# nintendops/DynamicFusion_Body

Measured on AMD Instinct MI355X. Metric: Mvoxels/s TSDF fusion + GN-iters/s warp solve, 256³ grid, 1/2/4/8 GPU, higher is better.
Workload: dtype f64 geometry / f32 volume

## Files before the change

dynamicfusion_body_amd/_lib.py:

```python
import ctypes
import os
import re

_PKG = os.path.dirname(os.path.abspath(__file__))
LIB_PATH = os.environ.get("DFH_LIB_PATH") or os.path.join(_PKG, "libdfusion_hip.so")
HEADER_PATH = os.path.join(os.path.dirname(_PKG), "include", "dfusion_hip.h")

F32, F64 = 0, 1
ABI_VERSION = 8

_c_double_p = ctypes.POINTER(ctypes.c_double)
_c_int_p = ctypes.POINTER(ctypes.c_int)
_vp = ctypes.c_void_p
_int = ctypes.c_int
_dbl = ctypes.c_double


class Problem(ctypes.Structure):
    _fields_ = [("sample_pos", _vp), ("sample_nrm", _vp), ("nbr", _vp), ("weights", _vp), ("corr", _vp), ("valid", _vp),
                ("n_samples", _int), ("knn", _int),
                ("node_dq", _vp), ("node_pos", _vp), ("node_w", _vp), ("node_nbr", _vp), ("n_nodes", _int),
                ("lw_dq", _dbl * 8), ("rw", _dbl), ("huber_delta", _dbl),
                ("row_ptr", _vp), ("col", _vp), ("n_blocks", _int), ("vals", _vp), ("rhs", _vp), ("cost_count", _vp),
                ("blk_upper", _vp), ("n_upper", _int),
# ... 13 lines not shown
                ("global_lm", _dbl), ("global_xi_out", _vp), ("global_scratch", _vp), ("global_scratch_bytes", ctypes.c_size_t)]


class Slab(ctypes.Structure):
    _fields_ = [("res", _int * 3), ("x0", _int), ("x1", _int)]


class Volume(ctypes.Structure):
    _fields_ = [("tsdf", _vp), ("tsdf_w", _vp), ("dtype", _int), ("slab", Slab)]


class Live(ctypes.Structure):
    _fields_ = [("data", _vp), ("dtype", _int), ("res", _int * 3)]


class VolumeTerm(ctypes.Structure):
    _fields_ = [("live", Live), ("value_to_vox", _dbl), ("band", _dbl), ("max_dist", _dbl), ("min_grad", _dbl)]


class DepthViews(ctypes.Structure):
    _fields_ = [("n_views", _int), ("depth", ctypes.POINTER(_vp)), ("depth_dtype", _int), ("H", _int), ("W", _int),
                ("K", _dbl * 9), ("Kinv", _dbl * 9), ("lw", _c_double_p), ("scale", _dbl), ("center", _dbl * 3), ("tsdf_res", _int)]


class Nodes(ctypes.Structure):
    _fields_ = [("pos", _vp), ("dq", _vp), ("w", _vp), ("n_nodes", _int), ("knn", _int)]


_problem_p = ctypes.POINTER(Problem)
_frame_p = ctypes.POINTER(Frame)
_slab_p = ctypes.POINTER(Slab)
_volume_p = ctypes.POINTER(Volume)
_term_p = ctypes.POINTER(VolumeTerm)
STRUCTS = {"dfh_gn_problem": Problem, "dfh_gn_frame": Frame, "dfh_gn_solve_params": SolveParams, "dfh_slab": Slab,
           "dfh_volume": Volume, "dfh_live": Live, "dfh_depth_views": DepthViews, "dfh_nodes": Nodes,
           "dfh_gn_volume_term": VolumeTerm}

_SIGNATURES = {
    "dfh_version": (_int, []),
    "dfh_last_error": (ctypes.c_char_p, []),
    "dfh_stream_synchronize": (_int, [_vp]),
    "dfh_set_option": (_int, [ctypes.c_char_p, ctypes.c_long]),
    "dfh_get_option": (ctypes.c_long, [ctypes.c_char_p]),
    "dfh_integrate_workspace_bytes": (ctypes.c_size_t, [_int, _int, _int, _slab_p]),
    "dfh_integrate_multi_workspace_bytes": (ctypes.c_size_t, [_int]),
    "dfh_integrate_depth": (_int, [_volume_p, ctypes.POINTER(DepthViews), _dbl, _dbl, _c_double_p, _vp, ctypes.c_size_t, _vp]),
    "dfh_integrate_depth_path": (_int, [_int, _slab_p, _int, _int, _int]),
    "dfh_integrate_depth_ocl": (_int, [_volume_p, _vp, _int, _int, ctypes.POINTER(ctypes.c_float), ctypes.POINTER(ctypes.c_float), ctypes.c_float, ctypes.c_float, _vp]),
    "dfh_fuse_volume_rigid": (_int, [_volume_p, ctypes.POINTER(Live), _c_double_p, _dbl, _dbl, _vp]),
    "dfh_dqb_workspace_bytes": (ctypes.c_size_t, [_slab_p]),
    "dfh_dqb_workspace_bytes_cached": (ctypes.c_size_t, [_slab_p, _int, _int, _int]),
    "dfh_fuse_volume_dqb": (_int, [_volume_p, ctypes.POINTER(Live), ctypes.POINTER(Nodes), _c_double_p, _dbl, _dbl, _vp, ctypes.c_size_t, _int, _vp]),
    "dfh_integrate_depth_dqb": (_int, [_volume_p, ctypes.POINTER(DepthViews), ctypes.POINTER(Nodes), _c_double_p, _dbl, _dbl, _int, _vp,
                                      ctypes.c_size_t, _int, _vp]),
    "dfh_residual_rigid": (_int, [_vp, _vp, _vp, _int, _c_double_p, _vp, _vp]),
    "dfh_gn_build_rigid": (_int, [_vp, _vp, _vp, _vp, _int, _c_double_p, _vp, _vp]),
    "dfh_residual_data": (_int, [_vp, _vp, _vp, _vp, _int, _int, _vp, _vp, _vp, _int, _c_double_p, _vp, _vp]),
    "dfh_residual_reg": (_int, [_vp, _int, _int, _vp, _vp, _vp, _dbl, _vp, _vp]),
    "dfh_warp_points": (_int, [_vp, _vp, _vp, _int, _int, _vp, _vp, _vp, _int, _c_double_p, _vp, _vp, _vp]),
    "dfh_closest_correspondences": (_int, [_vp, _vp, _int, _vp, _int, _int, _dbl, _vp, _vp, _vp, _vp]),
    "dfh_nearest_points": (_int, [_vp, _int, _vp, _int, _vp, _vp, _vp]),
    "dfh_graph_unsupported": (_int, [_vp, _int, _vp, _int, _vp, _vp, _int, _vp, _vp]),
    "dfh_dq_blend_points": (_int, [_vp, _int, _vp, _int, _vp, _vp, _vp, _int, _vp, _vp]),
    "dfh_radius_sample_workspace_bytes": (ctypes.c_size_t, [ctypes.c_long]),
    "dfh_radius_sample": (_int, [_vp, ctypes.c_long, _dbl, _vp, ctypes.c_long, ctypes.POINTER(ctypes.c_long), _c_int_p, _vp,
                                 ctypes.c_size_t, _vp]),
    "dfh_sample_knn": (_int, [_vp, _int, _vp, _vp, _int, _int, _vp, _vp, _vp]),
    "dfh_dqb_skip_layout": (_int, [_slab_p, _c_int_p, _int, _int, ctypes.POINTER(ctypes.c_size_t)]),
    "dfh_dqb_build_candidates": (_int, [_slab_p, _vp, _int, _int, _vp, ctypes.c_size_t, _vp]),
    "dfh_sample_knn_bricks": (_int, [_vp, _int, _vp, _vp, _int, _int, _slab_p, _vp, ctypes.c_size_t, _vp, _vp, _vp]),
    "dfh_permute_samples": (_int, [_vp, _int, _int, _vp, _vp, _vp, _vp, _vp, _vp, _vp, _vp, _vp]),
    "dfh_gn_partial_doubles": (ctypes.c_size_t, [_int]),
    "dfh_gn_views_bytes": (ctypes.c_size_t, [_int, _int, _int, _int]),
    "dfh_gn_pack_views": (_int, [_vp, _int, ctypes.POINTER(ctypes.c_void_p), _int, _int, _int, _c_double_p, _vp]),
    "dfh_gn_associate": (_int, [_problem_p, _frame_p, _vp]),
    "dfh_gn_associate_volume": (_int, [_problem_p, _term_p, _vp]),
    "dfh_gn_build": (_int, [_problem_p, _frame_p, _vp]),
    "dfh_gn_build_volume": (_int, [_problem_p, _term_p, _vp]),
    "dfh_gn_solve": (_int, [_problem_p, _frame_p, ctypes.POINTER(SolveParams), _vp]),
    "dfh_gn_solve_volume": (_int, [_problem_p, _term_p, ctypes.POINTER(SolveParams), _vp]),
    "dfh_gn_pack_upper": (_int, [_vp, _vp, _vp, _vp, _int, _int, _int, _vp, _vp]),
    "dfh_gn_unpack_upper": (_int, [_vp, _vp, _vp, _vp, _int, _int, _int, _vp, _vp]),
    "dfh_gn_sort_workspace_bytes": (ctypes.c_size_t, [_int]),
    "dfh_gn_sort_samples": (_int, [_vp, _vp, _vp, _vp, _int, _int, _int, _vp, _vp, _vp, _vp, _vp, _vp, _vp, ctypes.c_size_t, _vp]),
    "dfh_gn_tile_samples": (_int, []),
    "dfh_gn_plan_count": (_int, [_vp, _int, _int, _vp, _vp, _vp]),
    "dfh_gn_plan_workspace_bytes": (ctypes.c_size_t, [_int, _int]),
    "dfh_gn_plan_build": (_int, [_vp, _int, _int, _int, _vp, _int, _vp, _vp, _int, _vp, _vp, _vp, _vp, _vp, _vp, _vp, _vp,
                                 ctypes.c_size_t, _vp]),
    "dfh_pcg_workspace_bytes": (ctypes.c_size_t, [_int, _int]),
    "dfh_pcg_solve": (_int, [_vp, _vp, _vp, _vp, _int, _int, _dbl, _dbl, _vp, _vp, ctypes.c_size_t, _vp]),
    "dfh_pcg_solve_update": (_int, [_vp, _vp, _vp, _vp, _int, _int, _dbl, _dbl, _vp, _vp, ctypes.c_size_t, _vp, _dbl, _vp]),
    "dfh_pcg_set_mode": (_int, [_int]),
    "dfh_pcg_path": (_int, [_int]),
    "dfh_pcg_status": (_int, [_vp, ctypes.POINTER(ctypes.c_long)]),
    "dfh_pcg_status_peek": (_int, [_vp, ctypes.POINTER(ctypes.c_long)]),
    "dfh_apply_twist": (_int, [_vp, _vp, _int, _dbl, _vp]),
    "dfh_relax_twists": (_int, [_vp, _int, _dbl, _vp]),
    "dfh_gn_global_sampled_bytes": (ctypes.c_size_t, [_int, _int]),
    "dfh_gn_global_sampled": (_int, [_problem_p, _frame_p, _int, _dbl, _int, _vp, _vp, _vp, ctypes.c_size_t, _vp]),
    "dfh_gn_global_sampled_volume": (_int, [_problem_p, _term_p, _int, _dbl, _int, _vp, _vp, _vp, ctypes.c_size_t, _vp]),
    "dfh_gn_global_apply": (_int, [_vp, _dbl, _int, _vp, _vp, _vp]),
    "dfh_gn_global_step_bytes": (ctypes.c_size_t, []),
    "dfh_gn_global_step": (_int, [_vp, _int, _vp, _int, _dbl, _vp, _vp, _vp, ctypes.c_size_t, _vp]),
    "dfh_surface_workspace_bytes": (ctypes.c_size_t, [_c_int_p]),
    "dfh_surface_count": (_int, [_vp, _vp, _int, _c_int_p, _dbl, _vp, ctypes.c_size_t, _vp, _vp]),
    "dfh_surface_emit": (_int, [_vp, _vp, _int, _c_int_p, _int, _dbl, _vp, _vp, _vp, ctypes.c_long, _vp]),
    "dfh_mc_workspace_bytes": (ctypes.c_size_t, [_c_int_p, _int]),
    "dfh_mc_count": (_int, [_vp, _int, _c_int_p, _int, _dbl, _vp, ctypes.c_size_t, _vp, _vp]),
    "dfh_mc_emit": (_int, [_vp, _int, _c_int_p, _int, _dbl, _vp, ctypes.c_size_t, _vp, _vp, _vp, _vp, ctypes.c_long, ctypes.c_long,
                           ctypes.c_long, _vp]),
    "dfh_mc_reorder_workspace_bytes": (ctypes.c_size_t, [ctypes.c_long, ctypes.c_long]),
    "dfh_mc_reorder": (_int, [_vp, _vp, _vp, _vp, ctypes.c_long, ctypes.c_long, _vp, _vp, _vp, _vp, _vp, ctypes.c_size_t, _vp]),
    "dfh_render_workspace_bytes": (ctypes.c_size_t, [_int, _int, _int, ctypes.c_long]),
    "dfh_render_raster": (_int, [_vp, ctypes.c_long, _vp, ctypes.c_long, _int, _c_double_p, _c_double_p, _int, _int, _dbl, _c_double_p,
                                 _dbl, _dbl, _vp, ctypes.c_size_t, _vp]),
    "dfh_render_resolve": (_int, [_vp, _vp, ctypes.c_long, _vp, ctypes.c_long, _int, _c_double_p, _c_double_p, _int, _int, _dbl,
                                  _c_double_p, _dbl, _dbl, _vp, ctypes.c_size_t, _vp, _vp, _vp, _vp]),
}

_lib = None


class DfhError(RuntimeError):
    pass


class DfhTimeout(DfhError):
    """A persistent kernel gave up waiting in a grid barrier (DFH_E_TIMEOUT)."""


def declared_symbols(header=HEADER_PATH):
    txt = open(header).read()
    txt = re.sub(r"/\*.*?\*/", "", txt, flags=re.S)
    return sorted(set(re.findall(r"\b(dfh_[a-z0-9_]+)\s*\(", txt)))


def load():
    global _lib
    if _lib is not None:
        return _lib
    if not os.path.exists(LIB_PATH):
        raise DfhError("%s not found: the HIP library is the only implementation of this path "
                       "(no CPU fallback). Build it with `python -m dynamicfusion_body_amd.build`." % LIB_PATH)
    lib = ctypes.CDLL(LIB_PATH)
    for name, (res, args) in _SIGNATURES.items():
        fn = getattr(lib, name)
        fn.restype = res
        fn.argtypes = args
    v = lib.dfh_version()
    if v != ABI_VERSION:
        raise DfhError("libdfusion_hip.so ABI version %d != expected %d (rebuild)" % (v, ABI_VERSION))
    _lib = lib
    return lib


def check(rc, what):
    if rc != 0:
        msg = load().dfh_last_error().decode("utf-8", "replace")
        if rc == -1:
            raise ValueError("%s: %s" % (what, msg))
        if rc == -4:
            raise DfhTimeout("%s: %s" % (what, msg))
        raise DfhError("%s failed (%d): %s" % (what, rc, msg))


# ... 48 lines not shown
```

dynamicfusion_body_amd/csrc/dfh_common.h:

```cpp
#pragma once
#include <hip/hip_runtime.h>

#include <cstdarg>
#include <cstdio>

#include "../../include/dfusion_hip.h"

namespace dfh {

char *last_error_buf();
int fail(int code, const char *fmt, ...);

#define DFH_HIP_CHECK(expr)                                                               \
    do {                                                                                  \
        hipError_t _e = (expr);                                                           \
        if (_e != hipSuccess)                                                             \
            return ::dfh::fail(DFH_E_HIP, "%s failed: %s", #expr, hipGetErrorString(_e)); \
    } while (0)

#define DFH_REQUIRE(cond, ...)                                  \
    do {                                                        \
        if (!(cond)) return ::dfh::fail(DFH_E_BADARG, __VA_ARGS__); \
    } while (0)

inline int check_slab(const char *what, const dfh_slab *s) {
    DFH_REQUIRE(s, "%s: null slab", what);
    DFH_REQUIRE(s->res[0] > 0 && s->res[1] > 0 && s->res[2] > 0, "%s: bad grid %dx%dx%d", what, s->res[0], s->res[1], s->res[2]);
    DFH_REQUIRE(0 <= s->x0 && s->x0 <= s->x1 && s->x1 <= s->res[0], "%s: slab [%d,%d) outside [0,%d)", what, s->x0, s->x1, s->res[0]);
    DFH_REQUIRE(s->x1 - s->x0 <= 65535, "%s: slab has more than 65535 planes", what);
    return DFH_OK;
}

inline int check_volume(const char *what, const dfh_volume *v) {
    DFH_REQUIRE(v && v->tsdf && v->tsdf_w, "%s: null volume", what);
    DFH_REQUIRE(v->dtype == DFH_F32 || v->dtype == DFH_F64, "%s: bad volume dtype %d", what, v->dtype);
    return check_slab(what, &v->slab);
}

struct Mat3 { double m[9]; };
struct Mat34 { double m[12]; };
struct Vec3 { double v[3]; };
struct DQ { double q[8]; };

constexpr int kWave = 64;
#ifndef DFH_GN_TILE
#define DFH_GN_TILE 128
#endif
constexpr int kGnTile = DFH_GN_TILE;

#define DFH_OPTION_LIST(X)                                                                                                \
    X(k1_strided) X(k1_late_loads) X(k1_planes_per_block) X(k1_force_scalar) X(k1_bricks_min) X(k1_no_bricks)            \
    X(k1_bricks_nocull) X(k1_no_multi) X(k1_cull) X(k1_nzi) X(k1_prefetch) X(k1_nt) X(k1_gather_first)                  \
    X(k2_exact) X(k2_no_strided) X(k2_nt) X(k3_no_cache) X(k3_exact) X(k3_no_lds) X(k3_wg_per_cu) X(k3_tpb) X(k3_skip) X(plan_radix) X(rigid_atomic) X(gn_reg_own_launch) X(gn_reg_own_gather) \
    X(dbg_gather_part) X(pcg_wpb) X(pcg_multilaunch) X(pcg_spin_limit) X(pcg_one_xcd) X(gn_iter_own_clear) X(gn_gather_full) X(gn_no_view_cull)                                                            \
    X(py_plan_torch) X(py_allreduce_full) X(py_gn_atomic) X(py_gn_no_fused_assoc) X(py_gn_no_fused_iter) X(py_gn_iter_per_call) X(py_no_side_stream) X(py_no_host_scalars)
struct Options {
#define DFH_X(n) long n;
    DFH_OPTION_LIST(DFH_X)
#undef DFH_X
};
const Options &opt();

struct DeviceInfo {
    int n_cu = 0;
    int pcg_occ512 = -1, pcg_occ1024 = -1;
};
DeviceInfo &device_info(int device);
inline bool on(long v) { return v > 0; }

}
```

dynamicfusion_body_amd/csrc/dfh_plan.hip:

```cpp
#include "dfh_common.h"

#include <cstring>

#include <rocprim/device/device_radix_sort.hpp>

namespace dfh {

#ifndef DFH_SORT_BLOCK_ITEMS
#define DFH_SORT_BLOCK_ITEMS 8
#endif
using SortCfg = rocprim::radix_sort_config<rocprim::default_config,
                                           rocprim::merge_sort_config<512, 512, DFH_SORT_BLOCK_ITEMS, 128, 256, 8>,
                                           rocprim::default_config>;
constexpr int kPlanTile = kGnTile;
constexpr int kPlanWaves = kPlanTile / 64;
constexpr int kKMaxP = 8;

__device__ __forceinline__ int plan_find_block(const int *__restrict__ row_ptr, const int *__restrict__ col, int a, int b) {
    int lo = row_ptr[a], hi = row_ptr[a + 1] - 1;
    while (lo <= hi) {
        const int mid = (lo + hi) >> 1;
        const int c = col[mid];
        if (c == b) return mid;
        if (c < b) lo = mid + 1; else hi = mid - 1;
    }
    return -1;
}

__global__ __launch_bounds__(256) void plan_pack_keys_kernel(const int *__restrict__ nbr, int S, int k, unsigned long long N,
                                                              unsigned long long *__restrict__ key, int *__restrict__ idx) {
    const int s = blockIdx.x * 256 + threadIdx.x;
    if (s >= S) return;
    unsigned long long kk = 0;
    for (int j = 0; j < k; ++j) kk = kk * N + (unsigned long long)nbr[(size_t)s * k + j];
    key[s] = kk;
    idx[s] = s;
}

__global__ __launch_bounds__(256) void plan_permute_kernel(const int *__restrict__ order, int S, int k, const double *__restrict__ pos,
                                                           const double *__restrict__ nrm, const int *__restrict__ nbr,
                                                           const double *__restrict__ wts, double *__restrict__ pos_o,
                                                           double *__restrict__ nrm_o, int *__restrict__ nbr_o, double *__restrict__ wts_o) {
    const int i = blockIdx.x * 256 + threadIdx.x;
    if (i >= S) return;
    const size_t src = (size_t)order[i];
#pragma unroll
    for (int c = 0; c < 3; ++c) {
        pos_o[3 * (size_t)i + c] = pos[3 * src + c];
        nrm_o[3 * (size_t)i + c] = nrm[3 * src + c];
    }
    for (int j = 0; j < k; ++j) {
        nbr_o[(size_t)i * k + j] = nbr[src * k + j];
        wts_o[(size_t)i * k + j] = wts[src * k + j];
    }
}

__device__ __forceinline__ bool plan_is_head(const int *__restrict__ nbr, int s, int k) {
    if ((s & (kPlanTile - 1)) == 0) return true;
    bool h = false;
    for (int j = 0; j < k; ++j) h = h || nbr[(size_t)s * k + j] != nbr[(size_t)(s - 1) * k + j];
    return h;
}

__global__ __launch_bounds__(kPlanTile) void plan_heads_kernel(const int *__restrict__ nbr, int S, int k, int *__restrict__ tile_rows) {
    __shared__ int cnt[kPlanWaves];
    const int s = blockIdx.x * kPlanTile + threadIdx.x;
    const bool head = s < S && plan_is_head(nbr, s, k);
    const unsigned long long b = __ballot(head);
    if ((threadIdx.x & 63) == 0) cnt[threadIdx.x >> 6] = __popcll(b);
    __syncthreads();
    if (threadIdx.x == 0) {
        int n = 0;
        for (int w = 0; w < kPlanWaves; ++w) n += cnt[w];
        tile_rows[blockIdx.x] = n;
    }
}

__global__ __launch_bounds__(1024) void plan_scan_kernel(int *__restrict__ tile_rows, int n_tiles, int *__restrict__ n_rows_out) {
    __shared__ int wsum[16];
    __shared__ int carry_s;
    const int lane = threadIdx.x & 63, wv = threadIdx.x >> 6;
    if (threadIdx.x == 0) carry_s = 0;
    __syncthreads();
    for (int base = 0; base < n_tiles; base += 1024) {
        const int i = base + threadIdx.x;
        const int v = i < n_tiles ? tile_rows[i] : 0;
        int x = v;
#pragma unroll
        for (int o = 1; o < 64; o <<= 1) {
            const int y = __shfl_up(x, o, 64);
            if (lane >= o) x += y;
        }
        if (lane == 63) wsum[wv] = x;
        __syncthreads();
        int off = carry_s;
        for (int w = 0; w < wv; ++w) off += wsum[w];
        if (i < n_tiles) tile_rows[i] = off + x - v;
        __syncthreads();
        if (threadIdx.x == 1023) carry_s = off + x;
        __syncthreads();
    }
    if (threadIdx.x == 0) { tile_rows[n_tiles] = carry_s; *n_rows_out = carry_s; }
}

__global__ __launch_bounds__(kPlanTile) void plan_runid_kernel(const int *__restrict__ nbr, int S, int k, const int *__restrict__ tile_off,
                                                          int *__restrict__ run_id, int *__restrict__ row_first) {
    __shared__ int cnt[kPlanWaves];
    const int s = blockIdx.x * kPlanTile + threadIdx.x;
    const int lane = threadIdx.x & 63, wv = threadIdx.x >> 6;
    const bool head = s < S && plan_is_head(nbr, s, k);
    const unsigned long long b = __ballot(head);
    if (lane == 0) cnt[wv] = __popcll(b);
    __syncthreads();
    int r = tile_off[blockIdx.x] + __popcll(b & ((2ull << lane) - 1ull)) - 1;
    for (int w = 0; w < wv; ++w) r += cnt[w];
    if (s < S) {
        run_id[s] = r;
        if (head) row_first[r] = s;
    }
}

__device__ __forceinline__ int plan_count_slot(int *__restrict__ cnt, int key, bool active) {
    const int lane = threadIdx.x & 63;
    unsigned long long todo = __ballot(active);
    int leader = lane, rank = 0, size = 0;
    while (todo) {
        const int l0 = __ffsll((long long)todo) - 1;
        const int k0 = __shfl(key, l0, 64);
        const unsigned long long same = __ballot(active && key == k0) & todo;
        if (active && key == k0) {
            leader = l0;
            rank = __popcll(same & ((1ull << lane) - 1ull));
            size = __popcll(same);
        }
        todo &= ~same;
    }
// ... 124 lines not shown
                const int o = __shfl_xor(v, j, 64);
                const bool up = (lane & k) == 0, low = (lane & j) == 0;
                v = (low == up) ? min(v, o) : max(v, o);
            }
        if (lane < n) ent[beg + lane] = v;
        return;
    }
    if (n <= kListLds) {
        int P = 128;
        while (P < n) P <<= 1;
        int *a = sl[wv];
        for (int i = lane; i < P; i += 64) a[i] = i < n ? ent[beg + i] : kBig;
        for (int k = 2; k <= P; k <<= 1)
            for (int j = k >> 1; j > 0; j >>= 1) {
                __builtin_amdgcn_fence(__ATOMIC_RELEASE, "wavefront", "local");
                __builtin_amdgcn_wave_barrier();
                __builtin_amdgcn_fence(__ATOMIC_ACQUIRE, "wavefront", "local");
                for (int t = lane; t < P / 2; t += 64) {
                    const int i = ((t & ~(j - 1)) << 1) | (t & (j - 1));
                    const int x = a[i], y = a[i | j];
                    const bool up = (i & k) == 0;
                    if ((x > y) == up) { a[i] = y; a[i | j] = x; }
                }
            }
        __builtin_amdgcn_fence(__ATOMIC_RELEASE, "wavefront", "local");
        __builtin_amdgcn_wave_barrier();
        __builtin_amdgcn_fence(__ATOMIC_ACQUIRE, "wavefront", "local");
        for (int i = lane; i < n; i += 64) ent[beg + i] = a[i];
        return;
    }
    for (int i = lane; i < n; i += 64) tmp[beg + i] = ent[beg + i];
    __builtin_amdgcn_fence(__ATOMIC_RELEASE, "agent");
    __builtin_amdgcn_wave_barrier();
    __builtin_amdgcn_fence(__ATOMIC_ACQUIRE, "agent");
    for (int i = lane; i < n; i += 64) {
        const int x = tmp[beg + i];
        int r = 0;
        for (int q = 0; q < n; ++q) r += tmp[beg + q] < x ? 1 : 0;
        ent[beg + r] = x;
    }
}

__global__ __launch_bounds__(256) void plan_iota_kernel(int *__restrict__ a, long na, int *__restrict__ b, long nb) {
    const long i = (long)blockIdx.x * 256 + threadIdx.x;
    if (i < na) a[i] = (int)i;
    if (i < nb) b[i] = (int)i;
}

__global__ __launch_bounds__(256) void plan_ptr_kernel(const int *__restrict__ sorted, int n, int n_keys, int *__restrict__ ptr) {
    const int v = blockIdx.x * 256 + threadIdx.x;
    if (v > n_keys) return;
    int lo = 0, hi = n;
    while (lo < hi) {
        const int mid = (lo + hi) >> 1;
        if (sorted[mid] < v) lo = mid + 1; else hi = mid;
    }
    ptr[v] = lo;
}

static unsigned bits_for(unsigned long long max_value) {
    unsigned b = 1;
    while (b < 64 && (max_value >> b) != 0) ++b;
    return b;
}

static size_t align16(size_t x) { return (x + 15) / 16 * 16; }

static size_t sort_temp_bytes_u64(int n) {
    size_t t = 0;
    if (rocprim::radix_sort_pairs<SortCfg>(nullptr, t, (unsigned long long *)nullptr, (unsigned long long *)nullptr, (int *)nullptr, (int *)nullptr,
                                  (size_t)n) != hipSuccess) t = 0;
    return t;
}
static size_t sort_temp_bytes_i32(long n) {
    size_t t = 0;
    if (rocprim::radix_sort_pairs<SortCfg>(nullptr, t, (int *)nullptr, (int *)nullptr, (int *)nullptr, (int *)nullptr, (size_t)n) != hipSuccess) t = 0;
    return t;
}

}

extern "C" {

size_t dfh_gn_sort_workspace_bytes(int n_samples) {
    using namespace dfh;
    if (n_samples <= 0) return 0;
    return align16(sizeof(unsigned long long) * (size_t)n_samples) + align16(sizeof(int) * (size_t)n_samples) +
           align16(sort_temp_bytes_u64(n_samples));
}

int dfh_gn_sort_samples(const double *pos, const double *nrm, const int *nbr, const double *weights, int n_samples, int knn,
                        int n_nodes, double *pos_out, double *nrm_out, int *nbr_out, double *weights_out, long *key_out,
                        int *order_out, void *workspace, size_t workspace_bytes, void *stream) {
    using namespace dfh;
    DFH_REQUIRE(n_samples >= 0 && knn >= 1 && knn <= kKMaxP && n_nodes >= 1, "dfh_gn_sort_samples: bad sizes");
    if (n_samples == 0) return DFH_OK;
    DFH_REQUIRE(pos && nrm && nbr && weights && pos_out && nrm_out && nbr_out && weights_out && key_out && order_out && workspace,
                "dfh_gn_sort_samples: null pointer");
    DFH_REQUIRE(workspace_bytes >= dfh_gn_sort_workspace_bytes(n_samples), "dfh_gn_sort_samples: workspace too small");
    double span = 1.0;
    for (int j = 0; j < knn; ++j) span *= (double)n_nodes;
    DFH_REQUIRE(span < 9.0e18, "dfh_gn_sort_samples: %d digits in base %d do not fit 64 bits", knn, n_nodes);
    hipStream_t s = (hipStream_t)stream;
    char *w = static_cast<char *>(workspace);
    unsigned long long *key_in = reinterpret_cast<unsigned long long *>(w); w += align16(sizeof(unsigned long long) * (size_t)n_samples);
    int *idx_in = reinterpret_cast<int *>(w); w += align16(sizeof(int) * (size_t)n_samples);
    int *order = order_out;
    size_t temp = sort_temp_bytes_u64(n_samples);
    const dim3 grid((unsigned)((n_samples + 255) / 256)), block(256);
    hipLaunchKernelGGL(plan_pack_keys_kernel, grid, block, 0, s, nbr, n_samples, knn, (unsigned long long)n_nodes, key_in, idx_in);
    const unsigned end_bit = bits_for((unsigned long long)(span - 1.0) + 1ull);
    DFH_HIP_CHECK(rocprim::radix_sort_pairs<SortCfg>(w, temp, key_in, reinterpret_cast<unsigned long long *>(key_out), idx_in, order,
                                            (size_t)n_samples, 0u, end_bit > 64u ? 64u : end_bit, s));
    hipLaunchKernelGGL(plan_permute_kernel, grid, block, 0, s, order, n_samples, knn, pos, nrm, nbr, weights, pos_out, nrm_out, nbr_out,
                       weights_out);
    DFH_HIP_CHECK(hipGetLastError());
    return DFH_OK;
}

int dfh_gn_tile_samples(void) { return dfh::kGnTile; }

int dfh_gn_plan_count(const int *nbr, int n_samples, int knn, int *tile_off, int *n_rows_out, void *stream) {
    using namespace dfh;
    DFH_REQUIRE(n_samples >= 1 && knn >= 1 && knn <= kKMaxP, "dfh_gn_plan_count: bad sizes");
    DFH_REQUIRE(nbr && tile_off && n_rows_out, "dfh_gn_plan_count: null pointer");
    hipStream_t s = (hipStream_t)stream;
    const int n_tiles = (n_samples + kPlanTile - 1) / kPlanTile;
    hipLaunchKernelGGL(plan_heads_kernel, dim3(n_tiles), dim3(kPlanTile), 0, s, nbr, n_samples, knn, tile_off);
    hipLaunchKernelGGL(plan_scan_kernel, dim3(1), dim3(1024), 0, s, tile_off, n_tiles, n_rows_out);
    DFH_HIP_CHECK(hipGetLastError());
    return DFH_OK;
}

size_t dfh_gn_plan_workspace_bytes(int n_rows, int knn) {
    using namespace dfh;
    if (n_rows <= 0 || knn < 1 || knn > kKMaxP) return 0;
    const size_t E = (size_t)n_rows * knn * knn, E2 = (size_t)n_rows * knn;
    return 3 * align16(sizeof(int) * E) + 3 * align16(sizeof(int) * E2) + align16(sort_temp_bytes_i32((long)E)) + 16;
}

int dfh_gn_plan_build(const int *nbr, int n_samples, int knn, int n_nodes, const int *tile_off, int n_rows, const int *row_ptr,
                      const int *col, int n_blocks, int *run_id, int *row_first, int *blk_ptr, int *blk_ent, int *node_ptr,
                      int *node_ent, int *uncovered_out, void *workspace, size_t workspace_bytes, void *stream) {
    using namespace dfh;
    DFH_REQUIRE(n_samples >= 1 && knn >= 1 && knn <= kKMaxP && n_nodes >= 1 && n_blocks >= 1 && n_rows >= 1, "dfh_gn_plan_build: bad sizes");
    DFH_REQUIRE(nbr && tile_off && row_ptr && col && run_id && row_first && blk_ptr && blk_ent && node_ptr && node_ent && uncovered_out &&
                workspace, "dfh_gn_plan_build: null pointer");
    DFH_REQUIRE(workspace_bytes >= dfh_gn_plan_workspace_bytes(n_rows, knn), "dfh_gn_plan_build: workspace too small");
    DFH_REQUIRE((long)n_rows * knn * knn < (1L << 31), "dfh_gn_plan_build: too many rows for 32-bit entries");
    hipStream_t s = (hipStream_t)stream;
    const size_t E = (size_t)n_rows * knn * knn, E2 = (size_t)n_rows * knn;
    char *w = static_cast<char *>(workspace);
    int *bk_in = reinterpret_cast<int *>(w); w += align16(sizeof(int) * E);
    int *bv_in = reinterpret_cast<int *>(w); w += align16(sizeof(int) * E);
    int *bk_out = reinterpret_cast<int *>(w); w += align16(sizeof(int) * E);
    int *nk_in = reinterpret_cast<int *>(w); w += align16(sizeof(int) * E2);
    int *nv_in = reinterpret_cast<int *>(w); w += align16(sizeof(int) * E2);
    int *nk_out = reinterpret_cast<int *>(w); w += align16(sizeof(int) * E2);
    size_t temp = sort_temp_bytes_i32((long)E);
    int *unc_ws = reinterpret_cast<int *>(w + align16(temp));
    const int n_tiles = (n_samples + kPlanTile - 1) / kPlanTile;
    DFH_HIP_CHECK(hipMemsetAsync(unc_ws, 0, sizeof(int), s));
    hipLaunchKernelGGL(plan_runid_kernel, dim3(n_tiles), dim3(kPlanTile), 0, s, nbr, n_samples, knn, tile_off, run_id, row_first);
    if (on(opt().plan_radix)) {
        hipLaunchKernelGGL(plan_zero2_kernel, dim3((unsigned)((n_blocks + n_nodes + 2 + 255) / 256)), dim3(256), 0, s, blk_ptr, n_blocks + 1,
                           node_ptr, n_nodes + 1);
        hipLaunchKernelGGL(plan_keys_kernel, dim3((unsigned)((n_rows + 255) / 256), (unsigned)(knn * knn)), dim3(256), 0, s, nbr, row_first, n_rows, knn,
                           row_ptr, col, n_blocks, bk_in, bk_out, nk_in, nk_out, unc_ws, blk_ptr, node_ptr);
        hipLaunchKernelGGL(plan_flag_out_kernel, dim3(1), dim3(1), 0, s, unc_ws, uncovered_out);
        hipLaunchKernelGGL(plan_iota_kernel, dim3((unsigned)((E + 255) / 256)), dim3(256), 0, s, bv_in, (long)E, nv_in, (long)E2);
        DFH_HIP_CHECK(hipGetLastError());
        DFH_HIP_CHECK(rocprim::radix_sort_pairs<SortCfg>(w, temp, bk_in, bk_out, bv_in, blk_ent, E, 0u, bits_for((unsigned long long)n_blocks + 1ull), s));
        size_t temp2 = sort_temp_bytes_i32((long)E2);
        DFH_REQUIRE(temp2 <= temp, "dfh_gn_plan_build: scratch of the node sort exceeds the block sort's");
        DFH_HIP_CHECK(rocprim::radix_sort_pairs<SortCfg>(w, temp2, nk_in, nk_out, nv_in, node_ent, E2, 0u, bits_for((unsigned long long)n_nodes), s));
        hipLaunchKernelGGL(plan_ptr_kernel, dim3((unsigned)((n_blocks + 1 + 255) / 256)), dim3(256), 0, s, bk_out, (int)E, n_blocks, blk_ptr);
        hipLaunchKernelGGL(plan_ptr_kernel, dim3((unsigned)((n_nodes + 1 + 255) / 256)), dim3(256), 0, s, nk_out, (int)E2, n_nodes, node_ptr);
        DFH_HIP_CHECK(hipGetLastError());
        return DFH_OK;
    }
    hipLaunchKernelGGL(plan_zero2_kernel, dim3((unsigned)((n_blocks + n_nodes + 2 + 255) / 256)), dim3(256), 0, s, blk_ptr, n_blocks + 1,
                       node_ptr, n_nodes + 1);
    hipLaunchKernelGGL(plan_keys_kernel, dim3((unsigned)((n_rows + 255) / 256), (unsigned)(knn * knn)), dim3(256), 0, s, nbr, row_first, n_rows, knn,
                       row_ptr, col, n_blocks, bk_in, bv_in, nk_in, nv_in, unc_ws, blk_ptr, node_ptr);
    hipLaunchKernelGGL(plan_scan2_kernel, dim3(2), dim3(1024), 0, s, blk_ptr, n_blocks, node_ptr, n_nodes, unc_ws, uncovered_out);
    hipLaunchKernelGGL(plan_fill_kernel, dim3((unsigned)((E + 255) / 256)), dim3(256), 0, s, bk_in, bv_in, (long)E, n_blocks, blk_ptr, blk_ent,
                       nk_in, nv_in, (long)E2, node_ptr, node_ent);
    hipLaunchKernelGGL(plan_sort_lists_kernel, dim3((unsigned)((n_blocks + n_nodes + 3) / 4)), dim3(256), 0, s, blk_ptr, blk_ent, n_blocks,
                       node_ptr, node_ent, n_nodes, bk_out, nk_out);
    DFH_HIP_CHECK(hipGetLastError());
    (void)temp;
    return DFH_OK;
}

}
```

include/dfusion_hip.h:

```cpp
#ifndef DFUSION_HIP_H
#define DFUSION_HIP_H

#include <stddef.h>
#include <stdint.h>

#ifdef __cplusplus
extern "C" {
#endif

#define DFH_ABI_VERSION 8

#define DFH_F32 0
#define DFH_F64 1

#define DFH_OK 0
#define DFH_E_BADARG (-1)
#define DFH_E_HIP (-2)
#define DFH_E_UNSUPPORTED (-3)
#define DFH_E_TIMEOUT (-4)
#define DFH_E_INTERNAL (-5)

int dfh_version(void);

const char *dfh_last_error(void);
// ... 82 lines not shown

size_t dfh_radius_sample_workspace_bytes(long n_points);
int dfh_radius_sample(const double *points, long n_points, double radius, int *idx_out, long capacity, long *count_out,
                      int *rounds_out, void *workspace, size_t workspace_bytes, void *stream);

int dfh_permute_samples(const long *order, int n_samples, int knn, const double *pos, const double *nrm, const int *nbr,
                        const double *weights, double *pos_out, double *nrm_out, int *nbr_out, double *weights_out, void *stream);

typedef struct dfh_gn_problem {
    const double *sample_pos, *sample_nrm;
    const int *nbr;
    const double *weights;
    double *corr;
    unsigned char *valid;
    int n_samples, knn;
    double *node_dq;
    const double *node_pos, *node_w;
    const int *node_nbr;
    int n_nodes;
    double lw_dq[8];
    double rw, huber_delta;
    const int *row_ptr, *col;
    int n_blocks;
    double *vals, *rhs, *cost_count;
    const int *blk_upper;
    int n_upper;
    const int *run_id;
    int n_rows;
    double *partial;
    const int *blk_ptr, *blk_ent, *node_ptr, *node_ent;
    double *partial_reg;
    const int *rblk_ptr, *rblk_ent, *rnode_ptr, *rnode_ent;
} dfh_gn_problem;

typedef struct dfh_gn_frame {
    const void *views;
    int n_views, depth_dtype;
    int H, W;
    double K[9], Kinv[9];
    double scale;
    double center[3];
    double half;
    double max_dist;
} dfh_gn_frame;

typedef struct dfh_gn_solve_params {
    int pcg_iters;
    double lm_abs, lm_rel;
    double *x_out;
    void *pcg_workspace;
    size_t pcg_workspace_bytes;
    double step;
    int n_iters;
    int n_global;
    double global_lm;
    double *global_xi_out;
    void *global_scratch;
    size_t global_scratch_bytes;
} dfh_gn_solve_params;

#define DFH_GN_MAX_VIEWS 16
size_t dfh_gn_views_bytes(int n_views, int depth_dtype, int H, int W);
int dfh_gn_pack_views(void *out, int n_views, const void *const *depth, int depth_dtype, int H, int W, const double *lw_cam,
                      void *stream);

int dfh_gn_associate(const dfh_gn_problem *problem, const dfh_gn_frame *frame, void *stream);

typedef struct dfh_gn_volume_term {
    dfh_live live;
    double value_to_vox;
    double band;
    double max_dist;
    double min_grad;
} dfh_gn_volume_term;
int dfh_gn_associate_volume(const dfh_gn_problem *problem, const dfh_gn_volume_term *term, void *stream);

int dfh_gn_build(const dfh_gn_problem *problem, const dfh_gn_frame *frame, void *stream);
int dfh_gn_build_volume(const dfh_gn_problem *problem, const dfh_gn_volume_term *term, void *stream);
size_t dfh_gn_partial_doubles(int knn);

int dfh_gn_tile_samples(void);

size_t dfh_gn_sort_workspace_bytes(int n_samples);
int dfh_gn_sort_samples(const double *pos, const double *nrm, const int *nbr, const double *weights, int n_samples, int knn,
                        int n_nodes, double *pos_out, double *nrm_out, int *nbr_out, double *weights_out, long *key_out,
                        int *order_out, void *workspace, size_t workspace_bytes, void *stream);
int dfh_gn_plan_count(const int *nbr, int n_samples, int knn, int *tile_off, int *n_rows_out, void *stream);
size_t dfh_gn_plan_workspace_bytes(int n_rows, int knn);
int dfh_gn_plan_build(const int *nbr, int n_samples, int knn, int n_nodes, const int *tile_off, int n_rows, const int *row_ptr,
                      const int *col, int n_blocks, int *run_id, int *row_first, int *blk_ptr, int *blk_ent, int *node_ptr,
                      int *node_ent, int *uncovered_out, void *workspace, size_t workspace_bytes, void *stream);

size_t dfh_pcg_workspace_bytes(int n_nodes, int iters);
int dfh_pcg_solve(const int *row_ptr, const int *col, double *vals, const double *rhs, int n_nodes, int iters,
                  double lm_abs, double lm_rel, double *x_out, void *workspace, size_t workspace_bytes, void *stream);

int dfh_pcg_solve_update(const int *row_ptr, const int *col, double *vals, const double *rhs, int n_nodes, int iters,
                         double lm_abs, double lm_rel, double *x_out, void *workspace, size_t workspace_bytes, double *node_dq,
                         double step, void *stream);

int dfh_gn_solve(const dfh_gn_problem *problem, const dfh_gn_frame *frame, const dfh_gn_solve_params *params, void *stream);
int dfh_gn_solve_volume(const dfh_gn_problem *problem, const dfh_gn_volume_term *term, const dfh_gn_solve_params *params, void *stream);

int dfh_gn_pack_upper(const double *system, const int *row_of, const int *col, const int *src, int n_blocks, int n_nodes, int n_upper,
                      double *packed, void *stream);
int dfh_gn_unpack_upper(double *system, const int *row_of, const int *col, const int *src, int n_blocks, int n_nodes, int n_upper,
                        const double *packed, void *stream);

int dfh_pcg_set_mode(int mode);
int dfh_pcg_path(int n_nodes);
int dfh_pcg_status(void *stream, long *aborted_solves_out);
int dfh_pcg_status_peek(void *stream, long *aborted_solves_out);

int dfh_apply_twist(double *node_dq, const double *xi, int n_nodes, double step, void *stream);
int dfh_relax_twists(double *node_dq, int n_nodes, double factor, void *stream);
size_t dfh_gn_global_sampled_bytes(int n_samples, int stride);
int dfh_gn_global_sampled(const dfh_gn_problem *problem, const dfh_gn_frame *frame, int stride, double lm_rel, int n_steps,
                          double *xi_out, double *sums_out, void *scratch, size_t scratch_bytes, void *stream);
int dfh_gn_global_sampled_volume(const dfh_gn_problem *problem, const dfh_gn_volume_term *term, int stride, double lm_rel, int n_steps,
                                 double *xi_out, double *sums_out, void *scratch, size_t scratch_bytes, void *stream);
int dfh_gn_global_apply(const double *sums29, double lm_rel, int n_nodes, double *node_dq, double *xi_out, void *stream);
size_t dfh_gn_global_step_bytes(void);
int dfh_gn_global_step(const double *vals, int n_blocks, const double *rhs, int n_nodes, double lm_rel, double *node_dq, double *xi_out,
                       void *scratch, size_t scratch_bytes, void *stream);

size_t dfh_surface_workspace_bytes(const int res[3]);
int dfh_surface_count(const void *tsdf, const void *tsdf_w, int vol_dtype, const int res[3], double band, void *workspace,
                      size_t workspace_bytes, long *total_out, void *stream);
int dfh_surface_emit(const void *tsdf, const void *tsdf_w, int vol_dtype, const int res[3], int x0, double band,
                     const void *workspace, double *pos_out, double *nrm_out, long capacity, void *stream);

size_t dfh_mc_workspace_bytes(const int res[3], int step);
int dfh_mc_count(const void *vol, int vol_dtype, const int res[3], int step, double level, void *workspace,
                 size_t workspace_bytes, long *totals_out, void *stream);
int dfh_mc_emit(const void *vol, int vol_dtype, const int res[3], int step, double level, void *workspace,
                size_t workspace_bytes, float *verts, float *normals, float *values, int *faces, long cap_verts, long cap_faces,
                long n_active_tiles, void *stream);
size_t dfh_mc_reorder_workspace_bytes(long n_verts, long n_faces);
int dfh_mc_reorder(const float *verts_in, const float *normals_in, const float *values_in, int *faces, long n_verts, long n_faces,
                   float *verts_out, float *normals_out, float *values_out, long *used_out, void *workspace,
                   size_t workspace_bytes, void *stream);

size_t dfh_render_workspace_bytes(int n_views, int H, int W, long n_faces);
int dfh_render_raster(const double *verts, long n_verts, const int *faces, long n_faces, int n_views, const double *K, const double *lw,
                      int H, int W, double scale, const double center[3], double half, double znear, void *workspace,
                      size_t workspace_bytes, void *stream);
int dfh_render_resolve(const double *verts, const double *normals, long n_verts, const int *faces, long n_faces, int n_views,
                       const double *K, const double *lw, int H, int W, double scale, const double center[3], double half, double znear,
                       const void *workspace, size_t workspace_bytes, float *depth_out, int *face_out, float *normal_out, void *stream);

#ifdef __cplusplus
}
#endif
#endif
```

Before: 501,400.

## Replace radix sort of samples with bucketed bitonic sort and merge

Sorting samples by their neighbour-node key now uses a custom scheme: samples are bucketed on the leading neighbour indices, buckets of up to 4096 entries are bitonic-sorted in LDS, and oversized buckets are merged by rank via binary search. The permute of pos/nrm/nbr/weights is fused into the final emit. This targets the multi-pass rocprim radix sort and its separate permute kernel. It adds five launches, a serial single-block scan, and the rocprim path is kept as a fallback via an option or when samples exceed bucket capacity.

New measurement: 500,600. Within noise of the previous version (-0.2%).

```diff
diff --git a/dynamicfusion_body_amd/_lib.py b/dynamicfusion_body_amd/_lib.py
--- a/dynamicfusion_body_amd/_lib.py
+++ b/dynamicfusion_body_amd/_lib.py
@@ -119,6 +119,7 @@
     "dfh_gn_pack_upper": (_int, [_vp, _vp, _vp, _vp, _int, _int, _int, _vp, _vp]),
     "dfh_gn_unpack_upper": (_int, [_vp, _vp, _vp, _vp, _int, _int, _int, _vp, _vp]),
     "dfh_gn_sort_workspace_bytes": (ctypes.c_size_t, [_int]),
+    "dfh_gn_sort_bucket_capacity": (_int, []),
     "dfh_gn_sort_samples": (_int, [_vp, _vp, _vp, _vp, _int, _int, _int, _vp, _vp, _vp, _vp, _vp, _vp, _vp, ctypes.c_size_t, _vp]),
     "dfh_gn_tile_samples": (_int, []),
     "dfh_gn_plan_count": (_int, [_vp, _int, _int, _vp, _vp, _vp]),
diff --git a/dynamicfusion_body_amd/csrc/dfh_common.h b/dynamicfusion_body_amd/csrc/dfh_common.h
--- a/dynamicfusion_body_amd/csrc/dfh_common.h
+++ b/dynamicfusion_body_amd/csrc/dfh_common.h
@@ -51,7 +51,7 @@
 #define DFH_OPTION_LIST(X)                                                                                                \
     X(k1_strided) X(k1_late_loads) X(k1_planes_per_block) X(k1_force_scalar) X(k1_bricks_min) X(k1_no_bricks)            \
     X(k1_bricks_nocull) X(k1_no_multi) X(k1_cull) X(k1_nzi) X(k1_prefetch) X(k1_nt) X(k1_gather_first)                  \
-    X(k2_exact) X(k2_no_strided) X(k2_nt) X(k3_no_cache) X(k3_exact) X(k3_no_lds) X(k3_wg_per_cu) X(k3_tpb) X(k3_skip) X(plan_radix) X(rigid_atomic) X(gn_reg_own_launch) X(gn_reg_own_gather) \
+    X(k2_exact) X(k2_no_strided) X(k2_nt) X(k3_no_cache) X(k3_exact) X(k3_no_lds) X(k3_wg_per_cu) X(k3_tpb) X(k3_skip) X(plan_radix) X(plan_sort_lib) X(rigid_atomic) X(gn_reg_own_launch) X(gn_reg_own_gather) \
     X(dbg_gather_part) X(pcg_wpb) X(pcg_multilaunch) X(pcg_spin_limit) X(pcg_one_xcd) X(gn_iter_own_clear) X(gn_gather_full) X(gn_no_view_cull)                                                            \
     X(py_plan_torch) X(py_allreduce_full) X(py_gn_atomic) X(py_gn_no_fused_assoc) X(py_gn_no_fused_iter) X(py_gn_iter_per_call) X(py_no_side_stream) X(py_no_host_scalars)
 struct Options {
diff --git a/dynamicfusion_body_amd/csrc/dfh_plan.hip b/dynamicfusion_body_amd/csrc/dfh_plan.hip
--- a/dynamicfusion_body_amd/csrc/dfh_plan.hip
+++ b/dynamicfusion_body_amd/csrc/dfh_plan.hip
@@ -52,6 +52,351 @@
     for (int j = 0; j < k; ++j) {
         nbr_o[(size_t)i * k + j] = nbr[src * k + j];
         wts_o[(size_t)i * k + j] = wts[src * k + j];
+    }
+}
+
+constexpr int kSortCap = 4096;
+constexpr int kSortThreads = 512;
+constexpr int kSortMaxBins = 65536;
+constexpr int kSortHistBins = 4096;
+constexpr int kSortWg = 1024;
+
+__device__ __forceinline__ int plan_count_slot(int *__restrict__ cnt, int key, bool active);
+
+__device__ __forceinline__ unsigned long long sort_key_bin(const int *__restrict__ nbr, int s, int k, unsigned long long N, int d, int bins,
+                                                           int &bin) {
+    unsigned long long kk = 0, bb = 0;
+    for (int j = 0; j < k; ++j) {
+        kk = kk * N + (unsigned long long)nbr[(size_t)s * k + j];
+        if (j + 1 == d) bb = kk;
+    }
+    bin = bb < (unsigned long long)bins ? (int)bb : bins - 1;
+    return kk;
+}
+
+template <bool kLds>
+__global__ __launch_bounds__(kSortWg) void sort_count_kernel(const int *__restrict__ nbr, int S, int k, unsigned long long N, int d, int bins,
+                                                             int *__restrict__ cnt) {
+    __shared__ int h[kLds ? kSortHistBins : 1];
+    const int s = blockIdx.x * kSortWg + threadIdx.x;
+    int bin = 0;
+    if (s < S) sort_key_bin(nbr, s, k, N, d, bins, bin);
+    if (kLds) {
+        for (int b = threadIdx.x; b < bins; b += kSortWg) h[b] = 0;
+        __syncthreads();
+        if (s < S) atomicAdd(&h[bin], 1);
+        __syncthreads();
+        for (int b = threadIdx.x; b < bins; b += kSortWg) {
+            const int c = h[b];
+            if (c) atomicAdd(cnt + b, c);
+        }
+    } else {
+        plan_count_slot(cnt, bin, s < S);
+    }
+}
+
+__global__ __launch_bounds__(1024) void sort_scan_kernel(int *__restrict__ cnt, int bins, int *__restrict__ off, int *__restrict__ xoff) {
+    __shared__ int wsum[16], wxsum[16];
+    const int lane = threadIdx.x & 63, wv = threadIdx.x >> 6;
+    const int per = (bins + 1023) / 1024;
+    const int i0 = (int)threadIdx.x * per;
+    int sum = 0, xsum = 0;
+    for (int j = 0; j < per; ++j)
+        if (i0 + j < bins) {
+            const int c = cnt[i0 + j];
+            sum += c;
+            xsum += c > kSortCap ? (c - 1) / kSortCap : 0;
+        }
+    int x = sum, xx = xsum;
+#pragma unroll
+    for (int o = 1; o < 64; o <<= 1) {
+        const int y = __shfl_up(x, o, 64), yy = __shfl_up(xx, o, 64);
+        if (lane >= o) { x += y; xx += yy; }
+    }
+    if (lane == 63) { wsum[wv] = x; wxsum[wv] = xx; }
+    __syncthreads();
+    int run = x - sum, xrun = xx - xsum;
+    for (int w = 0; w < wv; ++w) { run += wsum[w]; xrun += wxsum[w]; }
+    if (threadIdx.x == 1023) { off[bins] = run + sum; xoff[bins] = xrun + xsum; }
+    for (int j = 0; j < per; ++j)
+        if (i0 + j < bins) {
+            const int c = cnt[i0 + j];
+            off[i0 + j] = run;
+            cnt[i0 + j] = run;
+            xoff[i0 + j] = xrun;
+            run += c;
+            xrun += c > kSortCap ? (c - 1) / kSortCap : 0;
+        }
+}
+
+template <bool kLds>
+__global__ __launch_bounds__(kSortWg) void sort_scatter_kernel(const int *__restrict__ nbr, int S, int k, unsigned long long N, int d, int bins,
+                                                               int *__restrict__ cursor, unsigned long long *__restrict__ skey,
+                                                               int *__restrict__ sidx) {
+    __shared__ int h[kLds ? kSortHistBins : 1];
+    const int s = blockIdx.x * kSortWg + threadIdx.x;
+    int bin = 0, slot = 0;
+    unsigned long long key = 0;
+    if (s < S) key = sort_key_bin(nbr, s, k, N, d, bins, bin);
+    if (kLds) {
+        for (int b = threadIdx.x; b < bins; b += kSortWg) h[b] = 0;
+        __syncthreads();
+        int r = 0;
+        if (s < S) r = atomicAdd(&h[bin], 1);
+        __syncthreads();
+        for (int b = threadIdx.x; b < bins; b += kSortWg) {
+            const int c = h[b];
+            if (c) h[b] = atomicAdd(cursor + b, c);
+        }
+        __syncthreads();
+        slot = h[bin] + r;
+    } else {
+        slot = plan_count_slot(cursor, bin, s < S);
+    }
+    if (s < S) {
+        skey[slot] = key;
+        sidx[slot] = s;
+    }
+}
+
+__device__ __forceinline__ bool sort_chunk_of(int wg, int bins, const int *__restrict__ off, const int *__restrict__ xoff, int &beg0, int &nb,
+                                              int &chunk) {
+    int b = wg;
+    chunk = 0;
+    if (wg >= bins) {
+        const int e = wg - bins;
+        if (e >= xoff[bins]) return false;
+        int lo = 0, hi = bins - 1;
+        while (lo < hi) {
+            const int mid = (lo + hi + 1) >> 1;
+            if (xoff[mid] <= e) lo = mid; else hi = mid - 1;
+        }
+        b = lo;
+        chunk = e - xoff[b] + 1;
+    }
+    beg0 = off[b];
+    nb = off[b + 1] - beg0;
+    return chunk * kSortCap < nb;
+}
+
+__device__ __forceinline__ bool sort_less(unsigned long long ka, int ia, unsigned long long kb, int ib) {
+    return ka < kb || (ka == kb && ia < ib);
+}
+
+__device__ __forceinline__ void sort_cx(unsigned long long &ka, int &ia, unsigned long long &kb, int &ib, bool up) {
+    if (sort_less(kb, ib, ka, ia) == up) {
+        const unsigned long long k = ka; ka = kb; kb = k;
+        const int i = ia; ia = ib; ib = i;
+    }
+}
+
+__device__ __forceinline__ void sort_emit(int dst, unsigned long long key, int src_, int k, const double *__restrict__ pos,
+                                          const double *__restrict__ nrm, const int *__restrict__ nbr, const double *__restrict__ wts,
+                                          double *__restrict__ pos_o, double *__restrict__ nrm_o, int *__restrict__ nbr_o,
+                                          double *__restrict__ wts_o, unsigned long long *__restrict__ key_o, int *__restrict__ order_o) {
+    const size_t src = (size_t)src_, i = (size_t)dst;
+    key_o[i] = key;
+    order_o[i] = src_;
+#pragma unroll
+    for (int c = 0; c < 3; ++c) {
+        pos_o[3 * i + c] = pos[3 * src + c];
+        nrm_o[3 * i + c] = nrm[3 * src + c];
+    }
+    for (int j = 0; j < k; ++j) {
+        nbr_o[i * k + j] = nbr[src * k + j];
+        wts_o[i * k + j] = wts[src * k + j];
+    }
+}
+
+__global__ __launch_bounds__(kSortThreads) void sort_chunks_kernel(int bins, const int *__restrict__ off, const int *__restrict__ xoff,
+                                                                   unsigned long long *__restrict__ skey, int *__restrict__ sidx, int k,
+                                                                   const double *__restrict__ pos, const double *__restrict__ nrm,
+                                                                   const int *__restrict__ nbr, const double *__restrict__ wts,
+                                                                   double *__restrict__ pos_o, double *__restrict__ nrm_o,
+                                                                   int *__restrict__ nbr_o, double *__restrict__ wts_o,
+                                                                   unsigned long long *__restrict__ key_o, int *__restrict__ order_o) {
+    __shared__ unsigned long long lk[kSortCap];
+    __shared__ int lv[kSortCap];
+    int beg0, nb, chunk;
+    if (!sort_chunk_of(blockIdx.x, bins, off, xoff, beg0, nb, chunk)) return;
+    const int beg = beg0 + chunk * kSortCap, n = min(kSortCap, nb - chunk * kSortCap);
+    const int tid = threadIdx.x;
+    int P = 2;
+    while (P < n) P <<= 1;
+    constexpr int kU = kSortCap / kSortThreads;
+    {
+        unsigned long long a[kU];
+        int b[kU];
+#pragma unroll
+        for (int u = 0; u < kU; ++u) {
+            const int i = tid + u * kSortThreads;
+            a[u] = i < n ? skey[beg + i] : ~0ull;
+            b[u] = i < n ? sidx[beg + i] : 0x7fffffff;
+        }
+#pragma unroll
+        for (int u = 0; u < kU; ++u) {
+            const int i = tid + u * kSortThreads;
+            if (i < P) { lk[i] = a[u]; lv[i] = b[u]; }
+        }
+    }
+    for (int kk = 2; kk <= P; kk <<= 1) {
+        int j = kk >> 1;
+        if (__popc(kk - 1) & 1) {
+            __syncthreads();
+            for (int t = tid; t < P / 2; t += kSortThreads) {
+                const int i = ((t & ~(j - 1)) << 1) | (t & (j - 1));
+                unsigned long long ka = lk[i], kb = lk[i | j];
+                int ia = lv[i], ib = lv[i | j];
+                if (sort_less(kb, ib, ka, ia) == ((i & kk) == 0)) { lk[i] = kb; lk[i | j] = ka; lv[i] = ib; lv[i | j] = ia; }
+            }
+            j >>= 1;
+        }
+        for (; j > 0; j >>= 2) {
+            const int h = j >> 1;
+            __syncthreads();
+            for (int t = tid; t < P / 4; t += kSortThreads) {
+                const int i = ((t & ~(h - 1)) << 2) | (t & (h - 1));
+                const bool up = (i & kk) == 0;
+                unsigned long long k0 = lk[i], k1 = lk[i + h], k2 = lk[i + 2 * h], k3 = lk[i + 3 * h];
+                int v0 = lv[i], v1 = lv[i + h], v2 = lv[i + 2 * h], v3 = lv[i + 3 * h];
+                sort_cx(k0, v0, k2, v2, up);
+                sort_cx(k1, v1, k3, v3, up);
+                sort_cx(k0, v0, k1, v1, up);
+                sort_cx(k2, v2, k3, v3, up);
+                lk[i] = k0; lk[i + h] = k1; lk[i + 2 * h] = k2; lk[i + 3 * h] = k3;
+                lv[i] = v0; lv[i + h] = v1; lv[i + 2 * h] = v2; lv[i + 3 * h] = v3;
+            }
+        }
+    }
+    __syncthreads();
+    if (nb > kSortCap) {
+        for (int i = tid; i < n; i += kSortThreads) { skey[beg + i] = lk[i]; sidx[beg + i] = lv[i]; }
+        return;
+    }
+    for (int i = tid; i < n; i += kSortThreads) { key_o[beg + i] = lk[i]; order_o[beg + i] = lv[i]; }
+    for (int e0 = tid; e0 < 3 * n; e0 += kU * kSortThreads) {
+        double a[kU], b[kU];
+#pragma unroll
+        for (int u = 0; u < kU; ++u) {
+            const int e = e0 + u * kSortThreads;
+            if (e < 3 * n) {
+                const int r = e / 3, c = e - 3 * r;
+                const size_t src = 3 * (size_t)lv[r] + c;
+                a[u] = pos[src];
+                b[u] = nrm[src];
+            }
+        }
+#pragma unroll
+        for (int u = 0; u < kU; ++u) {
+            const int e = e0 + u * kSortThreads;
+            if (e < 3 * n) {
+                const size_t dst = 3 * (size_t)beg + e;
+                pos_o[dst] = a[u];
+                nrm_o[dst] = b[u];
+            }
+        }
+    }
+    for (int e0 = tid; e0 < k * n; e0 += kU * kSortThreads) {
+        int a[kU];
+        double b[kU];
+#pragma unroll
+        for (int u = 0; u < kU; ++u) {
+            const int e = e0 + u * kSortThreads;
+            if (e < k * n) {
+                const int r = e / k, c = e - k * r;
+                const size_t src = (size_t)k * lv[r] + c;
+                a[u] = nbr[src];
+                b[u] = wts[src];
+            }
+        }
+#pragma unroll
+        for (int u = 0; u < kU; ++u) {
+            const int e = e0 + u * kSortThreads;
+            if (e < k * n) {
+                const size_t dst = (size_t)k * beg + e;
+                nbr_o[dst] = a[u];
+                wts_o[dst] = b[u];
+            }
+        }
+    }
+}
+
+__global__ __launch_bounds__(kSortWg) void sort_merge_kernel(int bins, const int *__restrict__ off, const int *__restrict__ xoff,
+                                                             const unsigned long long *__restrict__ skey, const int *__restrict__ sidx, int k,
+                                                             const double *__restrict__ pos, const double *__restrict__ nrm,
+                                                             const int *__restrict__ nbr, const double *__restrict__ wts,
+                                                             double *__restrict__ pos_o, double *__restrict__ nrm_o,
+                                                             int *__restrict__ nbr_o, double *__restrict__ wts_o,
+                                                             unsigned long long *__restrict__ key_o, int *__restrict__ order_o) {
+    int beg0, nb, chunk;
+    if (!sort_chunk_of(blockIdx.x, bins, off, xoff, beg0, nb, chunk)) return;
+    if (nb <= kSortCap) return;
+    const int lane = threadIdx.x & 63;
+    const int cbeg = chunk * kSortCap, cend = min(nb, cbeg + kSortCap);
+    const int q0 = cbeg + blockIdx.y * kSortWg + ((int)threadIdx.x & ~63);
+    if (q0 >= cend) return;
+    const int n_act = min(64, cend - q0);
+    const bool act = lane < n_act;
+    const int q = q0 + (act ? lane : n_act - 1);
+    const unsigned long long key = skey[beg0 + q];
+    const int idx = sidx[beg0 + q];
+    const unsigned long long key_f = __shfl(key, 0, 64), key_l = __shfl(key, n_act - 1, 64);
+    const int idx_f = __shfl(idx, 0, 64), idx_l = __shfl(idx, n_act - 1, 64);
+    int rank = q - cbeg;
+    const int n_chunks = (nb + kSortCap - 1) / kSortCap;
+    constexpr int kMergeWays = 8;
+    for (int cb = 0; cb < n_chunks; cb += 64) {
+        int lo_f, hi_f, lo_l, hi_l, first;
+        {
+            const int c = cb + lane;
+            const bool live = c < n_chunks && c != chunk;
+            first = live ? c * kSortCap : 0;
+            lo_f = lo_l = first;
+            hi_f = hi_l = live ? min(nb, first + kSortCap) : first;
+        }
+        while (lo_f < hi_f || lo_l < hi_l) {
+            const bool sf = lo_f < hi_f, sl = lo_l < hi_l;
+            const int mf = sf ? (lo_f + hi_f) >> 1 : 0, ml = sl ? (lo_l + hi_l) >> 1 : 0;
+            const unsigned long long kf = sf ? skey[beg0 + mf] : 0ull, kl = sl ? skey[beg0 + ml] : 0ull;
+            const int xf = sf ? sidx[beg0 + mf] : 0, xl = sl ? sidx[beg0 + ml] : 0;
+            if (sf) { if (sort_less(kf, xf, key_f, idx_f)) lo_f = mf + 1; else hi_f = mf; }
+            if (sl) { if (sort_less(kl, xl, key_l, idx_l)) lo_l = ml + 1; else hi_l = ml; }
+        }
+        for (int g0 = 0; g0 < min(64, n_chunks - cb); g0 += kMergeWays) {
+            int lo[kMergeWays], hi[kMergeWays];
+#pragma unroll
+            for (int g = 0; g < kMergeWays; ++g) {
+                lo[g] = __shfl(lo_f, g0 + g, 64);
+                hi[g] = __shfl(lo_l, g0 + g, 64);
+            }
+            bool open = true;
+            while (open) {
+                open = false;
+#pragma unroll
+                for (int g = 0; g < kMergeWays; ++g) {
+                    const bool live = lo[g] < hi[g];
+                    const int mid = live ? (lo[g] + hi[g]) >> 1 : 0;
+                    const unsigned long long km = live ? skey[beg0 + mid] : 0ull;
+                    const int im = live ? sidx[beg0 + mid] : 0;
+                    if (live) {
+                        if (sort_less(km, im, key, idx)) lo[g] = mid + 1; else hi[g] = mid;
+                    }
+                    open = open || lo[g] < hi[g];
+                }
+            }
+#pragma unroll
+            for (int g = 0; g < kMergeWays; ++g) rank += lo[g] - __shfl(first, g0 + g, 64);
+        }
+    }
+    if (act) sort_emit(beg0 + rank, key, idx, k, pos, nrm, nbr, wts, pos_o, nrm_o, nbr_o, wts_o, key_o, order_o);
+}
+
+static void sort_buckets(int S, int N, int knn, int &d, int &bins) {
+    d = 0;
+    bins = 1;
+    while (d < knn && N > 1 && (long)S > (long)bins * (kSortCap / 2) && (long)bins * N <= kSortMaxBins) {
+        bins *= N;
+        ++d;
     }
 }
 
@@ -342,12 +687,16 @@
 
 extern "C" {
 
+static size_t sort_tables_bytes() { return 3 * dfh::align16(sizeof(int) * ((size_t)dfh::kSortMaxBins + 1)); }
+
 size_t dfh_gn_sort_workspace_bytes(int n_samples) {
     using namespace dfh;
     if (n_samples <= 0) return 0;
-    return align16(sizeof(unsigned long long) * (size_t)n_samples) + align16(sizeof(int) * (size_t)n_samples) +
-           align16(sort_temp_bytes_u64(n_samples));
-}
+    const size_t temp = align16(sort_temp_bytes_u64(n_samples)), tables = sort_tables_bytes();
+    return align16(sizeof(unsigned long long) * (size_t)n_samples) + align16(sizeof(int) * (size_t)n_samples) + (temp > tables ? temp : tables);
+}
+
+int dfh_gn_sort_bucket_capacity(void) { return dfh::kSortCap; }
 
 int dfh_gn_sort_samples(const double *pos, const double *nrm, const int *nbr, const double *weights, int n_samples, int knn,
                         int n_nodes, double *pos_out, double *nrm_out, int *nbr_out, double *weights_out, long *key_out,
@@ -365,15 +714,42 @@
     char *w = static_cast<char *>(workspace);
     unsigned long long *key_in = reinterpret_cast<unsigned long long *>(w); w += align16(sizeof(unsigned long long) * (size_t)n_samples);
     int *idx_in = reinterpret_cast<int *>(w); w += align16(sizeof(int) * (size_t)n_samples);
-    int *order = order_out;
-    size_t temp = sort_temp_bytes_u64(n_samples);
-    const dim3 grid((unsigned)((n_samples + 255) / 256)), block(256);
-    hipLaunchKernelGGL(plan_pack_keys_kernel, grid, block, 0, s, nbr, n_samples, knn, (unsigned long long)n_nodes, key_in, idx_in);
-    const unsigned end_bit = bits_for((unsigned long long)(span - 1.0) + 1ull);
-    DFH_HIP_CHECK(rocprim::radix_sort_pairs<SortCfg>(w, temp, key_in, reinterpret_cast<unsigned long long *>(key_out), idx_in, order,
-                                            (size_t)n_samples, 0u, end_bit > 64u ? 64u : end_bit, s));
-    hipLaunchKernelGGL(plan_permute_kernel, grid, block, 0, s, order, n_samples, knn, pos, nrm, nbr, weights, pos_out, nrm_out, nbr_out,
-                       weights_out);
+    int d, bins;
+    sort_buckets(n_samples, n_nodes, knn, d, bins);
+    if (on(opt().plan_sort_lib) || (long)n_samples > (long)bins * kSortCap) {
+        int *order = order_out;
+        size_t temp = sort_temp_bytes_u64(n_samples);
+        const dim3 grid((unsigned)((n_samples + 255) / 256)), block(256);
+        hipLaunchKernelGGL(plan_pack_keys_kernel, grid, block, 0, s, nbr, n_samples, knn, (unsigned long long)n_nodes, key_in, idx_in);
+        const unsigned end_bit = bits_for((unsigned long long)(span - 1.0) + 1ull);
+        DFH_HIP_CHECK(rocprim::radix_sort_pairs<SortCfg>(w, temp, key_in, reinterpret_cast<unsigned long long *>(key_out), idx_in, order,
+                                                (size_t)n_samples, 0u, end_bit > 64u ? 64u : end_bit, s));
+        hipLaunchKernelGGL(plan_permute_kernel, grid, block, 0, s, order, n_samples, knn, pos, nrm, nbr, weights, pos_out, nrm_out, nbr_out,
+                           weights_out);
+        DFH_HIP_CHECK(hipGetLastError());
+        return DFH_OK;
+    }
+    int *cnt = reinterpret_cast<int *>(w); w += align16(sizeof(int) * ((size_t)kSortMaxBins + 1));
+    int *off = reinterpret_cast<int *>(w); w += align16(sizeof(int) * ((size_t)kSortMaxBins + 1));
+    int *xoff = reinterpret_cast<int *>(w);
+    unsigned long long *key_o = reinterpret_cast<unsigned long long *>(key_out);
+    const unsigned long long N = (unsigned long long)n_nodes;
+    const dim3 per_sample((unsigned)((n_samples + kSortWg - 1) / kSortWg));
+    const unsigned n_chunks = (unsigned)(bins + n_samples / kSortCap);
+    DFH_HIP_CHECK(hipMemsetAsync(cnt, 0, sizeof(int) * (size_t)bins, s));
+    if (bins <= kSortHistBins)
+        hipLaunchKernelGGL(sort_count_kernel<true>, per_sample, dim3(kSortWg), 0, s, nbr, n_samples, knn, N, d, bins, cnt);
+    else
+        hipLaunchKernelGGL(sort_count_kernel<false>, per_sample, dim3(kSortWg), 0, s, nbr, n_samples, knn, N, d, bins, cnt);
+    hipLaunchKernelGGL(sort_scan_kernel, dim3(1), dim3(1024), 0, s, cnt, bins, off, xoff);
+    if (bins <= kSortHistBins)
+        hipLaunchKernelGGL(sort_scatter_kernel<true>, per_sample, dim3(kSortWg), 0, s, nbr, n_samples, knn, N, d, bins, cnt, key_in, idx_in);
+    else
+        hipLaunchKernelGGL(sort_scatter_kernel<false>, per_sample, dim3(kSortWg), 0, s, nbr, n_samples, knn, N, d, bins, cnt, key_in, idx_in);
+    hipLaunchKernelGGL(sort_chunks_kernel, dim3(n_chunks), dim3(kSortThreads), 0, s, bins, off, xoff, key_in, idx_in, knn, pos, nrm, nbr, weights,
+                       pos_out, nrm_out, nbr_out, weights_out, key_o, order_out);
+    hipLaunchKernelGGL(sort_merge_kernel, dim3(n_chunks, kSortCap / kSortWg), dim3(kSortWg), 0, s, bins, off, xoff, key_in, idx_in, knn, pos, nrm,
+                       nbr, weights, pos_out, nrm_out, nbr_out, weights_out, key_o, order_out);
     DFH_HIP_CHECK(hipGetLastError());
     return DFH_OK;
 }
diff --git a/include/dfusion_hip.h b/include/dfusion_hip.h
--- a/include/dfusion_hip.h
+++ b/include/dfusion_hip.h
@@ -188,6 +188,7 @@
 int dfh_gn_tile_samples(void);
 
 size_t dfh_gn_sort_workspace_bytes(int n_samples);
+int dfh_gn_sort_bucket_capacity(void);
 int dfh_gn_sort_samples(const double *pos, const double *nrm, const int *nbr, const double *weights, int n_samples, int knn,
                         int n_nodes, double *pos_out, double *nrm_out, int *nbr_out, double *weights_out, long *key_out,
                         int *order_out, void *workspace, size_t workspace_bytes, void *stream);
```
